# dealii-X/portable-multigrid

Measured on NVIDIA B200. Metric: GDoF/s of one multigrid V-cycle (fine-level DoFs / time); operator-apply GDoF/s in apply_gdofs, higher is better.
Workload: dtype f64

## Files before the change

### include/pmg_kernels.h

```cpp
#ifndef PMG_KERNELS_H
#define PMG_KERNELS_H

#include <stdint.h>

#ifdef __cplusplus
extern "C" {
#endif

#define PMGK_MAX_N1 10

typedef struct pmgk_level {
  int dim;
  int degree;
  int nx, ny, nz;
  int Nx, Ny, Nz;
  unsigned faces;
  int z0, nzl;
  int cz_lo, cz_hi;
  int z_own_lo, z_own_hi;
  double h[3];
  double S[PMGK_MAX_N1 * PMGK_MAX_N1];
  double lam[PMGK_MAX_N1];
  double Mref[PMGK_MAX_N1 * PMGK_MAX_N1];
  double Kref[PMGK_MAX_N1 * PMGK_MAX_N1];
  const double *dinv_tab;
  const double *dinv_vec;
  int tile_variant;
  const double *coef;
  int coef_cz0;
  double Sq[PMGK_MAX_N1 * PMGK_MAX_N1];
  double Dco[PMGK_MAX_N1 * PMGK_MAX_N1];
} pmgk_level;

enum { PMGK_APPLY = 0, PMGK_RESIDUAL = 1, PMGK_CHEB_FIRST = 2, PMGK_CHEB_STEP = 3 };

int pmgk_apply(const pmgk_level *lv, int mode, const double *u, const double *b, const double *xold,
               double *out, double f1, double f2, void *stream);
enum { PMGK_PART_ALL = 0, PMGK_PART_INTERIOR = 1, PMGK_PART_BOUNDARY = 2 };
int pmgk_apply_part(const pmgk_level *lv, int mode, const double *u, const double *b, const double *xold,
                    double *out, double f1, double f2, int part, void *stream);
int pmgk_apply_splits(const pmgk_level *lv, int mode);
typedef struct pmgk_push {
  double *out_lower, *out_upper;
  int lower_z0, upper_z0;
  void *mailbox, *mailbox_lower, *mailbox_upper;
  int push, consume;
} pmgk_push;
int pmgk_apply_push(const pmgk_level *lv, int mode, const double *u, const double *b, const double *xold,
                    double *out, double f1, double f2, const pmgk_push *push, void *stream);
int pmgk_apply_can_push(const pmgk_level *lv, int mode);
int pmgk_apply_geometry(const pmgk_level *lv, int *grid, int *block, int *smem_bytes, int *n_chunks);

int64_t pmgk_var_coef_doubles(const pmgk_level *lv);
int pmgk_var_fill_coef(const pmgk_level *lv, int kind, const double *gq, const double *gw, double *coef, void *stream);
int pmgk_var_fill_dinv(const pmgk_level *lv, const double *S2, const double *G2, double *dinv, void *stream);

int pmgk_fill_dinv(const pmgk_level *lv, double *dinv, void *stream);
int pmgk_scale_dinv(const pmgk_level *lv, double f, const double *b, double *out, void *stream);

int pmgk_set(double *x, double a, int64_t n, void *stream);
int pmgk_copy(double *dst, const double *src, int64_t n, void *stream);
int pmgk_axpby(double *out, double a, const double *x, double b, const double *y, int64_t n, void *stream);
int pmgk_scale(double *x, double a, int64_t n, void *stream);
int pmgk_dot(const double *x, const double *y, int64_t n, double *result, double *work, void *stream);
int pmgk_sum(const double *x, int64_t n, double *result, double *work, void *stream);
int pmgk_dot_work_doubles(void);
int pmgk_cg_update_xr(double *x, double *r, const double *p, const double *Ap, const double *alpha_dev,
                      int64_t n, double *result, double *work, void *stream);
int pmgk_cg_update_p(double *p, const double *z, const double *beta_dev, int64_t n, void *stream);
int pmgk_scalar_div(double *out, const double *num, const double *den, void *stream);
int pmgk_outer3(double *out, const double *lx, const double *ly, const double *lz, int Nx, int Ny, int nz, void *stream);
int pmgk_set_mod11(double *x, int64_t first_global, int64_t n, void *stream);

typedef struct pmgk_coarse_level {
  const pmgk_level *lv;
  int cheb_degree;
  double theta, delta;
  double *sol, *rhs, *tmp, *res;
} pmgk_coarse_level;
int pmgk_coarse_cycle_supported(const pmgk_level *lv);
int pmgk_coarse_cycle(const pmgk_coarse_level *levels, int n_levels, int pre, int post, const double *P1d_host, void *stream);

int pmgk_prolongate_and_add(int kind, const pmgk_level *coarse, const pmgk_level *fine, const double *P1d,
                            double *dst_fine, const double *src_coarse, void *stream);
// ... 18 lines not shown
```

### portable-multigrid_b200/csrc/pmg_apply.cu

```cuda
#include "pmg_apply_tile.h"
#include "pmg_cuda_common.h"
#include "pmg_kernels.h"

template <class Tile>
struct PmgDeviceExec {
  typename Tile::ThreadState st;
  template <class F> __device__ __forceinline__ void for_each_thread(F f) { f((int)threadIdx.x, st); }
  __device__ __forceinline__ void sync() { __syncthreads(); }
};

template <int P, int BX, int BY, int MINB>
__global__ void __launch_bounds__(PmgApplyTile<P, BX, BY>::NT, MINB)
pmg_apply_kernel(const __grid_constant__ PmgApplyParams<P> p)
{
  using Tile = PmgApplyTile<P, BX, BY>;
  extern __shared__ double pmg_smem[];
  PmgDeviceExec<Tile> ex;
  const int b = blockIdx.x;
  const int tile_x = b % p.tiles_x;
  const int tile_y = (b / p.tiles_x) % p.tiles_y;
  const int chunk = b / (p.tiles_x * p.tiles_y);
  Tile::run(p, ex, pmg_smem, tile_x, tile_y, chunk);
}

// ... 156 lines not shown
  if (mode != PMGK_APPLY && !b) return PMG_ERR_ARG;
  if (u == out) return PMG_ERR_ARG;
  return dispatch(lv, mode, u, b, xold, out, f1, f2, (cudaStream_t)stream, nullptr, part);
}

thread_local const pmgk_push *pmg_tl_push = nullptr;

static bool plane_kernel_level(const pmgk_level *lv)
{
  const bool small_level = small_level_of(lv);
  return lv->dim == 3 && !lv->coef && lv->degree <= PMG_PLANE_MAX_DEGREE && (lv->tile_variant == 6 || (lv->tile_variant == 0 && !small_level));
}

extern "C" int pmgk_apply_can_push(const pmgk_level *lv, int mode)
{
  return lv && (mode == PMGK_RESIDUAL || mode == PMGK_CHEB_FIRST || mode == PMGK_CHEB_STEP) && plane_kernel_level(lv) && lv->cz_hi - lv->cz_lo >= 2;
}

extern "C" int pmgk_apply_push(const pmgk_level *lv, int mode, const double *u, const double *b, const double *xold,
                               double *out, double f1, double f2, const pmgk_push *push, void *stream)
{
  if (!lv || !u || !out || !push) return PMG_ERR_ARG;
  if (mode != PMGK_APPLY && !b) return PMG_ERR_ARG;
  if (u == out) return PMG_ERR_ARG;
  if (!pmgk_apply_can_push(lv, mode)) return PMG_ERR_UNSUPPORTED;
  pmg_tl_push = push;
  const int rc = dispatch(lv, mode, u, b, xold, out, f1, f2, (cudaStream_t)stream, nullptr);
  pmg_tl_push = nullptr;
  return rc;
}

extern "C" int pmgk_apply_splits(const pmgk_level *lv, int mode)
{
  int g[4] = {0, 0, 0, 0};
  if (!lv) return 0;
  return dispatch(lv, mode, (const double *)16, (const double *)16, nullptr, (double *)32, 0, 0, 0, g, PMGK_PART_INTERIOR) == 0;
}

extern "C" int pmgk_apply_geometry(const pmgk_level *lv, int *grid, int *block, int *smem_bytes, int *n_chunks)
{
  int g[4] = {0, 0, 0, 0};
  const int rc = dispatch(lv, 0, (const double *)8, nullptr, nullptr, (double *)16, 0, 0, 0, g);
  if (grid) *grid = g[0];
  if (block) *block = g[1];
  if (smem_bytes) *smem_bytes = g[2];
  if (n_chunks) *n_chunks = g[3];
  return rc;
}
```

### portable-multigrid_b200/csrc/pmg_apply_plane.h

```cpp
#pragma once
#include "pmg_apply_sweep.h"

#if defined(__CUDA_ARCH__)
#define PMG_OPAQUE_PTR(ptr) asm volatile("" : "+l"(ptr))
#else
#define PMG_OPAQUE_PTR(ptr) ((void)0)
#endif
PMG_HD double pmg_plane_ldg(const double *ptr)
{
#if defined(__CUDA_ARCH__)
  double v;
  asm volatile("ld.global.f64 %0, [%1];\n" : "=d"(v) : "l"(ptr) : "memory");
  return v;
#else
  return *ptr;
#endif
}
PMG_HD void pmg_plane_prefetch(const double *ptr, int level)
{
#if defined(__CUDA_ARCH__)
  if (level == 1) asm volatile("prefetch.global.L2 [%0];\n" ::"l"(ptr) : "memory");
  else asm volatile("prefetch.global.L1 [%0];\n" ::"l"(ptr) : "memory");
#else
  (void)ptr; (void)level;
#endif
}
PMG_HD void pmg_plane_cp_async8(double *smem, unsigned base32, unsigned byte_off, const double *src_global)
{
#if defined(__CUDA_ARCH__)
  (void)smem;
  asm volatile("cp.async.ca.shared.global [%0], [%1], 8;\n" ::"r"(base32 + byte_off), "l"(src_global) : "memory");
#else
  (void)base32;
  *(double *)((char *)smem + byte_off) = *src_global;
#endif
}
struct alignas(16) PmgPlanePair { double c, d; };

#if defined(__CUDA_ARCH__)
#define PMG_KEEP(v) asm volatile("" : "+r"(v))
#else
#define PMG_KEEP(v) ((void)0)
#endif
PMG_HD void pmg_plane_stg(double *ptr, double v)
{
#if defined(__CUDA_ARCH__)
  asm volatile("st.global.f64 [%0], %1;\n" ::"l"(ptr), "d"(v) : "memory");
#else
  *ptr = v;
#endif
}

enum { PMG_FUSED_FROM_LO = 8, PMG_FUSED_FROM_HI = 9, PMG_FUSED_EPOCH_LO = 10, PMG_FUSED_EPOCH_HI = 11, PMG_FUSED_TICKET_LO = 12, PMG_FUSED_TICKET_HI = 13,
       PMG_FUSED_ERROR = 14  };

template <int P, int BX, int BY, int NT_, int FM = -1, int UZ = 1, int LW_ = 0, int NU_ = 3, int EPF = 0, int PR = 1, int XS = 1, int PUSH = 0>
struct PmgPlaneTile {
  static constexpr int N1 = P + 1;
  static constexpr int NT = NT_;
  static constexpr int MODE_STEP0 = 4;
  static PMG_HD int mode_of(const PmgSweepParams<P> &p)
  {
    return FM >= 0 ? FM : (p.mode == PMG_MODE_CHEB_STEP && p.xold == nullptr) ? MODE_STEP0 : p.mode;
  }
  static constexpr int OX = BX * P, OY = BY * P;
  static constexpr int XW = OX + P + 1, YW = OY + P + 1;
  static constexpr int UP = XW;
  static constexpr int UPLANE = YW * UP;
  static constexpr int CP = OY | 1;
// ... 399 lines not shown
    }
    if (DIR && t.xextra && tid < ERW) {
      const int gy = t.cy0 * P + tid;
      if (gy < p.Ny && (tid < OY || (!t.virt_y && gy == p.Ny - 1))) {
        const int64_t g = eoff + (int64_t)tid * p.Nx + OX;
        const double uc = pmg_plane_ldg(p.u + g);
        const double bb = (MODE != PMG_MODE_APPLY) ? pmg_plane_ldg(p.b + g) : 0.0;
        const double xo = has_xo ? pmg_plane_ldg(p.xold + g) : 0.0;
        pmg_plane_stg(p.out + g, epi_value<MODE>(p, 0.0, uc, bb, xo, true, 1.0));
      }
    }
  }
  template <int MODE>
  static PMG_HD void epilogue_m(const PmgSweepParams<P> &p, const TileGeom &t, const ThreadState &st, const double *smem, int slot,
                                int gz, int64_t eoff, int tid)
  {
    if (t.dirxy || gz == t.zlo || gz == t.zhi) epilogue_t<MODE, true>(p, t, st, smem, slot, gz, eoff, tid);
    else epilogue_t<MODE, false>(p, t, st, smem, slot, gz, eoff, tid);
  }
  static PMG_HD void epilogue(const PmgSweepParams<P> &p, const TileGeom &t, const ThreadState &st, const double *smem, int slot,
                              int gz, int64_t eoff, int tid)
  {
    switch (mode_of(p)) {
      case PMG_MODE_APPLY: epilogue_m<PMG_MODE_APPLY>(p, t, st, smem, slot, gz, eoff, tid); break;
      case PMG_MODE_RESIDUAL: epilogue_m<PMG_MODE_RESIDUAL>(p, t, st, smem, slot, gz, eoff, tid); break;
      case PMG_MODE_CHEB_FIRST: epilogue_m<PMG_MODE_CHEB_FIRST>(p, t, st, smem, slot, gz, eoff, tid); break;
      case PMG_MODE_CHEB_STEP: epilogue_m<PMG_MODE_CHEB_STEP>(p, t, st, smem, slot, gz, eoff, tid); break;
      default: epilogue_m<MODE_STEP0>(p, t, st, smem, slot, gz, eoff, tid); break;
    }
  }

  struct March {
    int cz_first, cz_begin, cz_end;
    bool top;
    int cur;
    int us;
    int gz_last;
    int gz_stop;
    int fetch_max;
    int q_lo, q_hi;
    int64_t eq;
    unsigned base32;
  };
  struct Plan { int n; int q[2]; int os[2]; };
  static PMG_HD Plan plan_of(const March &mc, int gz)
  {
    Plan pl; pl.n = 0;
    const int q = gz - P - 1;
    if (q >= mc.q_lo && q < mc.q_hi) {
      const int lay = q / P, k = q - lay * P;
      pl.q[0] = q; pl.os[0] = (k == P - 1) ? P - 1 + ((lay + 1) & 1) : k; pl.n = 1;
    }
    if (mc.top && gz == mc.gz_stop) { pl.q[pl.n] = mc.cz_end * P; pl.os[pl.n] = NOB - 1; ++pl.n; }
    return pl;
  }

  template <bool GEN, class Exec>
  static PMG_HD void layer(const PmgSweepParams<P> &p, const TileGeom &t, Exec &ex, double *smem, March &mc, int L)
  {
    double *Ub = smem + U_OFFSET, *Cb = smem + C_OFFSET, *Ob = smem + O_OFFSET;
    const bool prev_layer = L > mc.cz_first, emit_layer = L - 1 >= mc.cz_begin;
#pragma unroll(UZ ? P : 1)
    for (int jz = 0; jz < P; ++jz) {
      const int gz = L * P + jz;
      if (GEN && gz > mc.gz_stop) break;
      const bool last = GEN && (gz == mc.gz_last);
      const bool drain = GEN && (gz > mc.gz_last);
      const bool zero = GEN && (gz == t.zlo || gz == t.zhi);
      const bool fetch = gz + ND <= mc.fetch_max;
      int fs = mc.us + ND; if (fs >= NU) fs -= NU;
      double *Ucur = Ub + mc.us * UPLANE;
      double *Ccur = Cb + mc.cur * 2 * CPLANE;
      Plan pl;
      if (GEN) pl = plan_of(mc, gz);
      else {
        const int q = gz - P - 1;
        pl.n = (q >= mc.q_lo && q < mc.q_hi) ? 1 : 0; pl.q[0] = q; pl.q[1] = 0; pl.os[1] = 0;
        pl.os[0] = (P == 1) ? ((L - 1) & 1) : (jz == 0) ? P - 1 + ((L - 1) & 1) : jz - 1;
      }
      ex.for_each_thread([&](int, ThreadState &st) {
        load_plane(p, st, t.plane, smem, mc.base32, fs, fetch);
        if (pl.n > 0 && !drain) epi_issue(p, t, st, pl.q[0], mc.eq);
        if (!zero && !drain) ysweep(p, st, Ucur, Ccur);
        load_wait();
      });
      ex.sync();
      ex.for_each_thread([&](int tid, ThreadState &st) {
        const bool has_prev = (jz == 0) && prev_layer;
        if (!drain) xzsweep(p, st, Ccur, Ob, jz, zero, has_prev, !last, has_prev && emit_layer, last && mc.top, L & 1);
#pragma unroll
        for (int i = 0; i < 2; ++i)
          if (i < pl.n) {
            const int64_t eo = mc.eq + (int64_t)(pl.q[i] - (gz - P - 1)) * t.plane;
            if (drain || i > 0) epi_issue(p, t, st, pl.q[i], eo);
            epilogue(p, t, st, smem, pl.os[i], pl.q[i], eo, tid);
          }
      });
      mc.cur ^= 1;
      mc.us = (mc.us + 1 == NU) ? 0 : mc.us + 1;
      mc.eq += t.plane;
    }
  }

  template <class Exec>
  static PMG_HD void run(const PmgSweepParams<P> &p, Exec &ex, double *smem, int tile_x, int tile_y, int chunk)
  {
    const TileGeom t = geom(p, tile_x, tile_y);
    March mc;
    mc.cz_begin = p.cz_lo + chunk * p.layers_per_chunk;
    mc.cz_end = mc.cz_begin + p.layers_per_chunk;
    if (mc.cz_end > p.cz_hi) mc.cz_end = p.cz_hi;
    if (mc.cz_begin >= mc.cz_end) return;
    const bool halo = (mc.cz_begin > 0) && ((mc.cz_begin - 1) * P >= p.z0);
    mc.cz_first = halo ? mc.cz_begin - 1 : mc.cz_begin;
    mc.top = (mc.cz_end == p.cz_hi) && (mc.cz_end * P < p.z_own_hi);
    const int gz_first = mc.cz_first * P;
    mc.cur = 0; mc.us = 0;
#if defined(__CUDA_ARCH__)
    mc.base32 = (unsigned)__cvta_generic_to_shared(smem);
    PMG_KEEP(mc.base32);
#else
    mc.base32 = 0;
#endif
    mc.gz_last = mc.cz_end * P;
    mc.gz_stop = mc.gz_last + P;
    mc.fetch_max = (t.zhi >= 0 && t.zhi <= mc.gz_last) ? t.zhi - 1 : mc.gz_last;
    mc.q_lo = mc.cz_begin * P > p.z_own_lo ? mc.cz_begin * P : p.z_own_lo;
    mc.q_hi = mc.cz_end * P < p.z_own_hi ? mc.cz_end * P : p.z_own_hi;
    mc.eq = (int64_t)(gz_first - P - 1 - p.z0) * t.plane + t.tile0;
    const double *up = p.u + (int64_t)(gz_first - p.z0) * t.plane;

    int l_wait = -1;
    if constexpr (PUSH != 0)
      if (mc.gz_last >= p.z_own_hi && p.z_own_hi < p.Nz && (p.consume & 1) && p.mb_hi) {
        l_wait = (p.z_own_hi - ND) / P;
        if (l_wait <= mc.cz_first) { ex.wait_flag(p.mb, PMG_FUSED_FROM_HI, PMG_FUSED_EPOCH_HI); l_wait = -1; }
      }
    ex.for_each_thread([&](int tid, ThreadState &st) { decode(p, t, tid, st, smem); st.ld_src = up + st.ld_off; });
    ex.sync();
    ex.for_each_thread([&](int, ThreadState &st) {
#pragma unroll
      for (int d = 0; d < ND; ++d) {
        const int gz = gz_first + d;
        load_plane(p, st, t.plane, smem, mc.base32, d, gz <= mc.fetch_max && gz != t.zlo);
      }
      load_wait();
    });
    ex.sync();
    for (int L = mc.cz_first; L * P <= mc.gz_stop; ++L) {
      if constexpr (PUSH != 0)
        if (L == l_wait) ex.wait_flag(p.mb, PMG_FUSED_FROM_HI, PMG_FUSED_EPOCH_HI);
      const bool fast = L < mc.cz_end && L * P > t.zlo && (t.zhi < 0 || L * P + P - 1 < t.zhi);
      if (fast) layer<false>(p, t, ex, smem, mc, L);
      else layer<true>(p, t, ex, smem, mc, L);
    }
  }
  template <class Exec>
  static PMG_HD void push_boundary(const PmgSweepParams<P> &p, Exec &ex, int tile_x, int tile_y, bool at_lo, bool at_hi)
  {
    const int x0 = tile_x * OX, y0 = tile_y * OY;
    const int x1 = (tile_x == p.tiles_x - 1 || x0 + OX > p.Nx) ? p.Nx : x0 + OX;
    const int y1 = (tile_y == p.tiles_y - 1 || y0 + OY > p.Ny) ? p.Ny : y0 + OY;
    if (x0 >= x1 || y0 >= y1) return;
    const int w = x1 - x0, n = w * (y1 - y0);
    const int64_t plane = (int64_t)p.Nx * p.Ny;
    ex.sync();
    ex.for_each_thread([&](int tid, ThreadState &) {
      if (at_lo && p.push_lo) {
        const int64_t base = (int64_t)(p.z_own_lo - p.z0) * plane;
        for (int e = tid; e < n; e += NT) {
          const int r = e / w, c = e - r * w;
          const int64_t g = base + (int64_t)(y0 + r) * p.Nx + x0 + c;
          p.push_lo[g] = p.out[g];
        }
      }
      if (at_hi && p.push_hi) {
        for (int q = p.z_own_hi - P; q < p.z_own_hi; ++q) {
          const int64_t base = (int64_t)(q - p.z0) * plane;
          for (int e = tid; e < n; e += NT) {
            const int r = e / w, c = e - r * w;
            const int64_t g = base + (int64_t)(y0 + r) * p.Nx + x0 + c;
            p.push_hi[g] = p.out[g];
          }
        }
      }
// ... 9 lines not shown
```

### portable-multigrid_b200/csrc/pmg_apply_plane_launch.h

```cpp
#include "pmg_apply_plane.h"
#include "pmg_cuda_common.h"
#include "pmg_kernels.h"

namespace {

__device__ __forceinline__ void pmg_st_release_sys(unsigned long long *p, unsigned long long v)
{
  asm volatile("st.release.sys.global.u64 [%0], %1;\n" ::"l"(p), "l"(v) : "memory");
}
__device__ __forceinline__ unsigned long long pmg_ld_acquire_sys(const unsigned long long *p)
{
  unsigned long long v;
  asm volatile("ld.acquire.sys.global.u64 %0, [%1];\n" : "=l"(v) : "l"(p) : "memory");
  return v;
}

template <class Tile>
struct PmgPlaneDeviceExec {
  typename Tile::ThreadState st;
  template <class F> __device__ __forceinline__ void for_each_thread(F f) { f((int)threadIdx.x, st); }
  __device__ __forceinline__ void sync() { __syncthreads(); }
  __device__ __forceinline__ void wait_flag(unsigned long long *mb, int flag, int epoch)
  {
    if (threadIdx.x == 0) {
      const unsigned long long e = pmg_ld_acquire_sys(mb + epoch);
      if (pmg_ld_acquire_sys(mb + flag) < e) {
        const long long t0 = clock64();
        while (pmg_ld_acquire_sys(mb + flag) < e && pmg_ld_acquire_sys(mb + PMG_FUSED_ERROR) == 0) {
          __nanosleep(100);
          if (clock64() - t0 > 8000000000ll) { atomicExch(mb + PMG_FUSED_ERROR, 1ull); break; }
        }
      }
    }
    __syncthreads();
  }
};

template <int P, int BX, int BY, int NT, int MINB, int UZ, int FM, int PR, int XS, int PUSH>
__global__ void __launch_bounds__(NT, MINB)
pmg_plane_kernel(const __grid_constant__ PmgSweepParams<P> p, int chunk_first, int chunk_stride)
{
  using Tile = PmgPlaneTile<P, BX, BY, NT, FM, UZ, 0, 3, 0, PR, XS, PUSH>;
  extern __shared__ __align__(128) double pmg_plane_smem[];
  PmgPlaneDeviceExec<Tile> ex;
  const int b = blockIdx.x;
  const int tile_x = b % p.tiles_x;
  const int tile_y = (b / p.tiles_x) % p.tiles_y;
  const int group = b / (p.tiles_x * p.tiles_y);
  int chunk = chunk_first + group * chunk_stride;
  bool at_lo = false, at_hi = false;
  if (PUSH && p.mb) {
    const int last = p.n_chunks - 1;
    if (!(p.consume & 2)) chunk = group == 0 ? last : group == last ? 0 : group;
    at_lo = chunk == 0; at_hi = chunk == last;
    if (at_lo && (p.consume & 1) && p.mb_lo) ex.wait_flag(p.mb, PMG_FUSED_FROM_LO, PMG_FUSED_EPOCH_LO);
  }
  Tile::run(p, ex, pmg_plane_smem, tile_x, tile_y, chunk);
  if (!PUSH || !(at_lo || at_hi)) return;
  Tile::push_boundary(p, ex, tile_x, tile_y, at_lo, at_hi);
  __syncthreads();
  if (threadIdx.x == 0) {
    if (p.consume & 8) __threadfence(); else if (!(p.consume & 4)) __threadfence_system();
    const unsigned long long tiles = (unsigned long long)p.tiles_x * p.tiles_y;
    if (at_lo && atomicAdd(p.mb + PMG_FUSED_TICKET_LO, 1ull) == tiles - 1) {
      p.mb[PMG_FUSED_TICKET_LO] = 0;
      const unsigned long long e = pmg_ld_acquire_sys(p.mb + PMG_FUSED_EPOCH_LO) + 1;
      __threadfence_system();
      if (p.mb_lo) pmg_st_release_sys(p.mb_lo + PMG_FUSED_FROM_HI, e);
      pmg_st_release_sys(p.mb + PMG_FUSED_EPOCH_LO, e);
    }
    if (at_hi && atomicAdd(p.mb + PMG_FUSED_TICKET_HI, 1ull) == tiles - 1) {
      p.mb[PMG_FUSED_TICKET_HI] = 0;
      const unsigned long long e = pmg_ld_acquire_sys(p.mb + PMG_FUSED_EPOCH_HI) + 1;
      __threadfence_system();
      if (p.mb_hi) pmg_st_release_sys(p.mb_hi + PMG_FUSED_FROM_LO, e);
      pmg_st_release_sys(p.mb + PMG_FUSED_EPOCH_HI, e);
    }
  }
}

inline void choose_plane_chunks(int tiles, int layers, int slots, int degree, int *n_chunks, int *layers_per_chunk)
{
  const long c_target = (8L * slots + tiles - 1) / tiles;
  const long c_fill = (slots + tiles - 1) / tiles;
  const int lpc_min = (32 + degree - 1) / degree;
  long c_cap = layers / lpc_min;
  long c_fill_cap = layers / 2;
  if (c_cap < 1) c_cap = 1;
  if (c_fill_cap < 1) c_fill_cap = 1;
  long c_floor = c_fill < c_fill_cap ? c_fill : c_fill_cap;
  if (c_floor < c_cap) c_floor = c_cap;
  long c = c_target < c_floor ? c_target : c_floor;
  if (c < 1) c = 1;
  const int lpc = (layers + (int)c - 1) / (int)c;
  *layers_per_chunk = lpc;
  *n_chunks = (layers + lpc - 1) / lpc;
}

template <int P, int BX, int BY, int NT, int MINB, int UZ, int FM, int PR, int XS, int PUSH>
int launch_plane(const pmgk_level *lv, const double *u, const double *b, const double *xold, double *out, double f1, double f2,
                 cudaStream_t stream, int *geom, int part)
{
  using Tile = PmgPlaneTile<P, BX, BY, NT, FM, UZ, 0, 3, 0, PR, XS, PUSH>;
  auto kernel = pmg_plane_kernel<P, BX, BY, NT, MINB, UZ, FM, PR, XS, PUSH>;
  PmgSweepParams<P> p;
  p.nx = lv->nx; p.ny = lv->ny; p.nz = lv->nz;
  p.Nx = lv->Nx; p.Ny = lv->Ny; p.Nz = lv->Nz;
  p.faces = lv->faces;
  p.z0 = lv->z0; p.nzl = lv->nzl;
  p.cz_lo = lv->cz_lo; p.cz_hi = lv->cz_hi;
  p.z_own_lo = lv->z_own_lo; p.z_own_hi = lv->z_own_hi;
  p.tiles_x = Tile::tiles_of(lv->nx, lv->faces >> 1 & 1u, BX);
  p.tiles_y = Tile::tiles_of(lv->ny, lv->faces >> 3 & 1u, BY);
  const int smem_bytes = Tile::SMEM_DOUBLES * (int)sizeof(double);
  enum { MAXDEV = 64 };
  static int ctas_per_sm[MAXDEV];
  int dev = 0;
  PMG_CUDA_CHECK(cudaGetDevice(&dev));
  if (dev < 0 || dev >= MAXDEV) return PMG_ERR_UNSUPPORTED;
  int per_sm = __atomic_load_n(&ctas_per_sm[dev], __ATOMIC_ACQUIRE);
  if (per_sm == 0) {
    PMG_CUDA_CHECK(cudaFuncSetAttribute(kernel, cudaFuncAttributeMaxDynamicSharedMemorySize, smem_bytes));
    PMG_CUDA_CHECK(cudaOccupancyMaxActiveBlocksPerMultiprocessor(&per_sm, kernel, NT, smem_bytes));
    if (per_sm < 1) return PMG_ERR_CUDA;
    __atomic_store_n(&ctas_per_sm[dev], per_sm, __ATOMIC_RELEASE);
  }
  const int slots = pmgk_device_sm_count() * per_sm;
  choose_plane_chunks(p.tiles_x * p.tiles_y, lv->cz_hi - lv->cz_lo, slots, P, &p.n_chunks, &p.layers_per_chunk);
  pmg_sweep_fill_matrices<P>(p, lv->Mref, lv->Kref, lv->h);
  p.mode = (FM == 4) ? PMG_MODE_CHEB_STEP : FM; p.u = u; p.b = b; p.xold = xold; p.out = out; p.f1 = f1; p.f2 = f2;
  p.dinv_vec = lv->dinv_vec; p.dinv_tab = lv->dinv_tab;
  p.push_lo = p.push_hi = nullptr; p.mb = p.mb_lo = p.mb_hi = nullptr; p.consume = 0;
  if (const pmgk_push *ps = PUSH ? pmg_tl_push : nullptr) {
    if (part != PMGK_PART_ALL || lv->cz_hi - lv->cz_lo < 2 || !ps->mailbox) return PMG_ERR_UNSUPPORTED;
    const int64_t plane = (int64_t)lv->Nx * lv->Ny;
    if (ps->push && ps->out_lower) p.push_lo = ps->out_lower + plane * (lv->z0 - ps->lower_z0);
    if (ps->push && ps->out_upper) p.push_hi = ps->out_upper + plane * (lv->z0 - ps->upper_z0);
    p.mb = (unsigned long long *)ps->mailbox;
    p.mb_lo = (unsigned long long *)ps->mailbox_lower; p.mb_hi = (unsigned long long *)ps->mailbox_upper;
    p.consume = ps->consume;
  }
  int chunk_first = 0, chunk_stride = 1, chunk_count = p.n_chunks;
  if (part != PMGK_PART_ALL) {
    if (p.n_chunks < 3) return PMG_ERR_UNSUPPORTED;
    if (part == PMGK_PART_INTERIOR) { chunk_first = 1; chunk_count = p.n_chunks - 2; }
    else { chunk_stride = p.n_chunks - 1; chunk_count = 2; }
  }
  const int grid = p.tiles_x * p.tiles_y * chunk_count;
  if (geom) { geom[0] = grid; geom[1] = NT; geom[2] = smem_bytes; geom[3] = p.n_chunks; return 0; }
  if ((int64_t)lv->Nx * lv->Ny * 4 >= (int64_t)1 << 31) return PMG_ERR_UNSUPPORTED;
  kernel<<<grid, NT, smem_bytes, stream>>>(p, chunk_first, chunk_stride);
  PMG_CUDA_CHECK(cudaGetLastError());
  pmg_count_launch(1);
  return 0;
}

}

#define PMG_PLANE_CAT2(a, b) a##b
#define PMG_PLANE_CAT(a, b) PMG_PLANE_CAT2(a, b)

int PMG_PLANE_CAT(pmg_plane_dispatch_m, PMG_PLANE_TU_MODE)(const pmgk_level *lv, const double *u, const double *b, const double *xold,
                                                           double *out, double f1, double f2, cudaStream_t s, int *geom, int part)
{
  switch (lv->degree) {
#if PMG_PLANE_TU_MODE >= 1
#define PMG_PLANE_LAUNCH(P, BX, BY, NT, MINB, UZ, PR, XS)                                                                              \
  case P:                                                                                                                             \
    return pmg_tl_push ? launch_plane<P, BX, BY, NT, MINB, UZ, PMG_PLANE_TU_MODE, PR, XS, 1>(lv, u, b, xold, out, f1, f2, s, geom, part) \
                       : launch_plane<P, BX, BY, NT, MINB, UZ, PMG_PLANE_TU_MODE, PR, XS, 0>(lv, u, b, xold, out, f1, f2, s, geom, part);
#else
#define PMG_PLANE_LAUNCH(P, BX, BY, NT, MINB, UZ, PR, XS) \
  case P: return pmg_tl_push ? PMG_ERR_UNSUPPORTED : launch_plane<P, BX, BY, NT, MINB, UZ, PMG_PLANE_TU_MODE, PR, XS, 0>(lv, u, b, xold, out, f1, f2, s, geom, part);
#endif
#if PMG_PLANE_TU_MODE == 0
#define PMG_PLANE_CASE(P, BX, BY, NT, MINB, UZ, PR, XS) PMG_PLANE_LAUNCH(P, BX, BY, NT, MINB, UZ, PR, XS)
#define PMG_PLANE_CASE_F(P, BX, BY, NT, MINB, UZ, PR, XS)
#else
#define PMG_PLANE_CASE(P, BX, BY, NT, MINB, UZ, PR, XS)
#define PMG_PLANE_CASE_F(P, BX, BY, NT, MINB, UZ, PR, XS) PMG_PLANE_LAUNCH(P, BX, BY, NT, MINB, UZ, PR, XS)
#endif
#include "pmg_apply_plane_tiles.inc"
#undef PMG_PLANE_CASE
// ... 6 lines not shown
```

### portable-multigrid_b200/csrc/pmg_apply_sweep.h

```cpp
#pragma once
#include <stdint.h>
#include <math.h>

#if defined(__CUDACC__)
#define PMG_HD __host__ __device__ __forceinline__
#else
#define PMG_HD inline
#endif

#ifndef PMG_APPLY_MODES_DEFINED
#define PMG_APPLY_MODES_DEFINED
enum PmgApplyMode {
  PMG_MODE_APPLY = 0,
  PMG_MODE_RESIDUAL = 1,
  PMG_MODE_CHEB_FIRST = 2,
  PMG_MODE_CHEB_STEP = 3,
};
#endif

PMG_HD void pmg_mbar_init(uint64_t *bar, int count)
{
#if defined(__CUDA_ARCH__)
  asm volatile("mbarrier.init.shared::cta.b64 [%0], %1;\n" ::"r"((unsigned)__cvta_generic_to_shared(bar)), "r"(count) : "memory");
#else
// ... 47 lines not shown
{
#if defined(__CUDA_ARCH__)
  asm volatile("cp.async.bulk.shared::cluster.global.mbarrier::complete_tx::bytes [%0], [%1], %2, [%3];\n"
               ::"r"((unsigned)__cvta_generic_to_shared(dst_smem)), "l"(src_global), "r"(bytes),
                 "r"((unsigned)__cvta_generic_to_shared(bar)) : "memory");
#else
  (void)bar;
  for (int i = 0; i < bytes / 8; ++i) dst_smem[i] = src_global[i];
#endif
}

template <int P>
struct PmgSweepParams {
  int nx, ny, nz;
  int Nx, Ny, Nz;
  unsigned faces;
  int z0, nzl;
  int cz_lo, cz_hi;
  int z_own_lo, z_own_hi;
  int tiles_x, tiles_y, n_chunks, layers_per_chunk;
  double M[(P + 1) * (P + 1)], Kx[(P + 1) * (P + 1)], Ky[(P + 1) * (P + 1)];
  double Mz[(P + 1) * (P + 1)], Kz[(P + 1) * (P + 1)];
  int mode;
  const double *u;
  const double *b;
  const double *xold;
  double *out;
  double f1, f2;
  const double *dinv_vec;
  const double *dinv_tab;
  double *push_lo, *push_hi;
  unsigned long long *mb, *mb_lo, *mb_hi;
  int consume;
};

template <int P>
inline void pmg_sweep_fill_matrices(PmgSweepParams<P> &p, const double *Mref, const double *Kref, const double *h)
{
  constexpr int N1 = P + 1;
  const double cx = h[1] * h[2] / h[0], cy = h[0] * h[2] / h[1], cz = h[0] * h[1] / h[2];
  for (int i = 0; i < N1; ++i)
    for (int j = 0; j < N1; ++j) {
      const int a = i * N1 + j, b = j * N1 + i, c = (P - i) * N1 + (P - j), d = (P - j) * N1 + (P - i);
      const double m = 0.25 * (Mref[a] + Mref[b] + Mref[c] + Mref[d]);
      const double k = 0.25 * (Kref[a] + Kref[b] + Kref[c] + Kref[d]);
      p.M[a] = m; p.Kx[a] = k; p.Ky[a] = (cy / cx) * k; p.Mz[a] = cx * m; p.Kz[a] = cz * k;
    }
}

template <int P>
PMG_HD int pmg_sweep_pos_type(int g, int N)
{
  return (g == 0) ? P : (g == N - 1) ? P + 1 : g % P;
}

template <int P>
PMG_HD constexpr int pmg_sweep_canon(int i, int j)
{
  int m = i * (P + 1) + j;
  const int b = j * (P + 1) + i, c = (P - i) * (P + 1) + (P - j), d = (P - j) * (P + 1) + (P - i);
  if (b < m) m = b;
  if (c < m) m = c;
  if (d < m) m = d;
  return m;
}

// ... 631 lines not shown
```

### portable-multigrid_b200/host/pmg_internal.h

```cpp
#ifndef PMG_INTERNAL_H
#define PMG_INTERNAL_H

#include <cuda_runtime_api.h>
#include <nccl.h>
#include <stdint.h>
#include "pmg.h"
#include "pmg_kernels.h"

#ifdef __cplusplus
extern "C" {
#endif

void pmg_set_error(const char *fmt, ...);
void pmg_count_launch(int n);
int pmg_enter(const pmg_context *ctx);

#define PMG_CHECK(call)                        \
  do {                                         \
    int pmg_rc_ = (call);                      \
    if (pmg_rc_ != PMG_OK) return pmg_rc_;     \
  } while (0)

#define PMG_CUDA(call)                                                                            \
  do {                                                                                            \
// ... 83 lines not shown
  int gathered;
  int cz_lo, cz_hi;
  int z0, nzl;
  int z_own_lo, z_own_hi;
  int lower, upper;
  int64_t plane;
  int64_t n_local;
  int64_t n_global;
} pmg_layout;

int pmg_p2p_init(pmg_context *ctx);
void pmg_p2p_shutdown(pmg_context *ctx);
int pmg_p2p_register(pmg_context *ctx, const pmg_layout *lay, double *d);
double *pmg_p2p_acquire(pmg_context *ctx, const pmg_layout *lay);
int pmg_p2p_release(pmg_context *ctx, double *d);
int pmg_p2p_halo(pmg_context *ctx, const pmg_layout *lay, double *d, cudaStream_t stream, int *done);
void pmg_p2p_forget(pmg_context *ctx);
int pmg_p2p_push_desc(pmg_context *ctx, const pmg_layout *lay, double *out, pmgk_push *desc);

struct pmg_vector {
  pmg_context *ctx;
  pmg_layout lay;
  double *d;
  int borrowed;
};

struct pmg_operator {
  pmg_context *ctx;
  int dim, degree, coefficient;
  unsigned faces;
  pmg_layout lay;
  pmgk_level lv;
  double *d_dinv_tab;
  double *d_coef;
  pmg_vector *dinv;
  pmg_vector *cg_ws[4];
};

struct pmg_transfer {
  pmg_context *ctx;
  int kind;
  const pmg_operator *coarse, *fine;
  double *d_P;
  double *d_scratch;
  pmg_vector *gather_buf;
};

struct pmg_chebyshev {
  pmg_operator *op;
  double smoothing_range;
  int degree, eig_cg_n_iterations;
  int initialized;
  double lambda_min, lambda_max, theta, delta;
  int cg_iterations;
  pmg_vector *t0, *t1;
};

int pmg_layout_make(pmg_context *ctx, int dim, int degree, int nx, int ny, int nz, pmg_layout *lay);
int pmg_layout_same(const pmg_layout *a, const pmg_layout *b);
int pmg_vector_create_layout(pmg_context *ctx, const pmg_layout *lay, pmg_vector **v);
int pmg_halo_update(pmg_context *ctx, const pmg_layout *lay, double *d);
int pmg_halo_update_on(pmg_context *ctx, const pmg_layout *lay, double *d, ncclComm_t comm, cudaStream_t stream);
int pmg_allreduce_sum(pmg_context *ctx, double *dev_scalar, int count);
int pmg_vector_dot_device(const pmg_vector *x, const pmg_vector *y, int slot);
int pmg_apply_with_halo(const pmg_operator *op, int mode, double *u, const double *b, const double *xold, double *out, double f1, double f2);
int pmg_apply_chain_ok(const pmg_operator *op, int mode, double *v0, double *v1);
// ... 13 lines not shown
```

### portable-multigrid_b200/host/pmg_operator.c

```c
#include "pmg_internal.h"
#include <math.h>
#include <stdlib.h>
#include <string.h>

static int var_diagonal(pmg_operator *op)
{
  const int n1 = op->degree + 1;
  double Sq[PMGK_MAX_N1 * PMGK_MAX_N1], G[PMGK_MAX_N1 * PMGK_MAX_N1];
  pmg_fe_shape_tables(op->degree, Sq, NULL, G, NULL, NULL);
  for (int i = 0; i < n1 * n1; ++i) { Sq[i] *= Sq[i]; G[i] *= G[i]; }
  return pmgk_var_fill_dinv(&op->lv, Sq, G, op->dinv->d, op->ctx->stream);
}

static int setup_coefficient(pmg_operator *op)
{
  pmgk_level *lv = &op->lv;
  double gq[PMGK_MAX_N1], gw[PMGK_MAX_N1];
  pmg_fe_shape_tables(op->degree, lv->Sq, lv->Dco, NULL, gq, gw);
  lv->coef_cz0 = lv->z0 / op->degree;
  PMG_CHECK(pmg_vector_create_layout(op->ctx, &op->lay, &op->dinv));
  if (!op->lay.active) return PMG_OK;
  const int64_t n = pmgk_var_coef_doubles(lv);
  if (cudaMalloc((void **)&op->d_coef, sizeof(double) * (size_t)n) != cudaSuccess) {
    pmg_set_error("cudaMalloc of %lld coefficient values failed", (long long)n);
// ... 19 lines not shown
  pmg_operator *op = (pmg_operator *)calloc(1, sizeof(*op));
  if (!op) return PMG_ERR_NOMEM;
  op->ctx = ctx; op->dim = dim; op->degree = degree; op->coefficient = coefficient; op->faces = faces & PMG_ALL_FACES;
  PMG_CHECK(pmg_layout_make(ctx, dim, degree, nx, ny, nz, &op->lay));
  pmgk_level *lv = &op->lv;
  lv->dim = dim;
  lv->degree = degree;
  lv->nx = nx; lv->ny = ny; lv->nz = nz;
  lv->Nx = op->lay.Nx; lv->Ny = op->lay.Ny; lv->Nz = op->lay.Nz;
  lv->faces = op->faces;
  lv->z0 = op->lay.z0; lv->nzl = op->lay.nzl;
  lv->cz_lo = op->lay.cz_lo; lv->cz_hi = op->lay.cz_hi;
  lv->z_own_lo = op->lay.z_own_lo; lv->z_own_hi = op->lay.z_own_hi;
  lv->h[0] = 1.0 / nx; lv->h[1] = 1.0 / ny; lv->h[2] = (dim == 2) ? 1.0 : 1.0 / nz;
  pmg_fe_fastdiag(degree, lv->S, lv->lam);
  pmg_fe_pencil(degree, lv->Mref, lv->Kref);
  const int T = degree + 2;
  double *tab = (double *)malloc(sizeof(double) * T * T * T);
  if (!tab) { free(op); return PMG_ERR_NOMEM; }
  pmg_fe_dinv_table(degree, lv->h, dim, tab);
  PMG_CUDA(cudaSetDevice(ctx->device));
  PMG_CUDA(cudaMalloc((void **)&op->d_dinv_tab, sizeof(double) * T * T * T));
  PMG_CUDA(cudaMemcpyAsync(op->d_dinv_tab, tab, sizeof(double) * T * T * T, cudaMemcpyHostToDevice, ctx->stream));
  PMG_CUDA(cudaStreamSynchronize(ctx->stream));
  free(tab);
  lv->dinv_tab = op->d_dinv_tab;
  lv->dinv_vec = NULL;
  const char *tv = getenv("PMG_TILE_VARIANT");
  lv->tile_variant = tv ? atoi(tv) : 0;
  if (coefficient != 0) {
    const int rc = setup_coefficient(op);
    if (rc != PMG_OK) { pmg_laplace_operator_destroy(op); return rc; }
  }
  *out = op;
  return PMG_OK;
}

int pmg_laplace_operator_destroy(pmg_operator *op)
{
  if (!op) return PMG_OK;
  cudaStreamSynchronize(op->ctx->stream);
  if (op->dinv) pmg_vector_destroy(op->dinv);
  for (int i = 0; i < 4; ++i) if (op->cg_ws[i]) pmg_vector_destroy(op->cg_ws[i]);
  cudaFree(op->d_dinv_tab);
  cudaFree(op->d_coef);
  free(op);
  return PMG_OK;
}

static int check_vec(const pmg_operator *op, const pmg_vector *v, const char *what)
{
  if (!v || v->ctx != op->ctx || !pmg_layout_same(&v->lay, &op->lay)) {
    pmg_set_error("%s: vector is not initialised for this operator (initialize_dof_vector)", what);
    return PMG_ERR_ARG;
  }
  return PMG_OK;
}

static int fused_order_bit(void)
{
  static int natural_order = -1;
  if (natural_order < 0) { const char *e = getenv("PMG_FUSED_ORDER"); natural_order = (e && atoi(e) == 1) ? 0 : 1; }
  return natural_order ? 2 : 0;
}

int pmg_apply_with_halo(const pmg_operator *op, int mode, double *u, const double *b, const double *xold, double *out, double f1, double f2)
{
  if (op) PMG_CHECK(pmg_enter(op->ctx));
  pmg_context *ctx = op->ctx;
  if (!op->lay.active) return PMG_OK;
  const int slab = ctx->has_comm && !op->lay.gathered;
  if (slab && ctx->overlap && pmgk_apply_splits(&op->lv, mode)) {
    PMG_CUDA(cudaEventRecord(ctx->ev_ready, ctx->stream));
    PMG_CUDA(cudaStreamWaitEvent(ctx->halo_stream, ctx->ev_ready, 0));
    PMG_CHECK(pmg_halo_update_on(ctx, &op->lay, u, ctx->halo_comm, ctx->halo_stream));
    PMG_CUDA(cudaEventRecord(ctx->ev_halo, ctx->halo_stream));
    PMG_CHECK(pmgk_apply_part(&op->lv, mode, u, b, xold, out, f1, f2, PMGK_PART_INTERIOR, ctx->stream));
// ... 234 lines not shown
```

Measured before the change: 3.118.

## Add dynamic persistent work-claiming scheduler for plane sweep kernel chunks

For non-push full applies, the plane kernel now launches at most one CTA per resident slot. Each CTA claims (tile, chunk) items from a global atomic counter in a staggered run order. When a CTA reaches the end of its chunk it can claim the next chunk of the same tile and keep marching, which reuses the plane data already in shared memory instead of reloading halo layers. Chunks are made shorter to give finer load balance. This adds atomic traffic, a grid-wide reset of the schedule table by the last CTA, and a per-operator device buffer.

```diff
diff --git a/include/pmg_kernels.h b/include/pmg_kernels.h
--- a/include/pmg_kernels.h
+++ b/include/pmg_kernels.h
@@ -25,6 +25,8 @@
   double Kref[PMGK_MAX_N1 * PMGK_MAX_N1];
   const double *dinv_tab;
   const double *dinv_vec;
+  int *plane_sched;
+  int64_t plane_sched_words;
   int tile_variant;
   const double *coef;
   int coef_cz0;
@@ -50,6 +52,7 @@
                     double *out, double f1, double f2, const pmgk_push *push, void *stream);
 int pmgk_apply_can_push(const pmgk_level *lv, int mode);
 int pmgk_apply_geometry(const pmgk_level *lv, int *grid, int *block, int *smem_bytes, int *n_chunks);
+int64_t pmgk_plane_sched_words(const pmgk_level *lv);
 
 int64_t pmgk_var_coef_doubles(const pmgk_level *lv);
 int pmgk_var_fill_coef(const pmgk_level *lv, int kind, const double *gq, const double *gw, double *coef, void *stream);
diff --git a/portable-multigrid_b200/csrc/pmg_apply.cu b/portable-multigrid_b200/csrc/pmg_apply.cu
--- a/portable-multigrid_b200/csrc/pmg_apply.cu
+++ b/portable-multigrid_b200/csrc/pmg_apply.cu
@@ -212,14 +212,28 @@
 
 extern "C" int pmgk_apply_splits(const pmgk_level *lv, int mode)
 {
-  int g[4] = {0, 0, 0, 0};
+  int g[5] = {0, 0, 0, 0, 0};
   if (!lv) return 0;
   return dispatch(lv, mode, (const double *)16, (const double *)16, nullptr, (double *)32, 0, 0, 0, g, PMGK_PART_INTERIOR) == 0;
 }
 
+extern "C" int64_t pmgk_plane_sched_words(const pmgk_level *lv)
+{
+  int64_t words = 0;
+  if (!lv) return 0;
+  for (int mode = PMGK_APPLY; mode <= PMGK_CHEB_STEP + 1; ++mode) {
+    int g[5] = {0, 0, 0, 0, 0};
+    const int m = mode > PMGK_CHEB_STEP ? PMGK_CHEB_STEP : mode;
+    if (dispatch(lv, m, (const double *)8, (const double *)8, mode == PMGK_CHEB_STEP ? (const double *)8 : nullptr, (double *)16, 0, 0, 0, g) == 0 &&
+        g[4] > words)
+      words = g[4];
+  }
+  return words;
+}
+
 extern "C" int pmgk_apply_geometry(const pmgk_level *lv, int *grid, int *block, int *smem_bytes, int *n_chunks)
 {
-  int g[4] = {0, 0, 0, 0};
+  int g[5] = {0, 0, 0, 0, 0};
   const int rc = dispatch(lv, 0, (const double *)8, nullptr, nullptr, (double *)16, 0, 0, 0, g);
   if (grid) *grid = g[0];
   if (block) *block = g[1];
diff --git a/portable-multigrid_b200/csrc/pmg_apply_plane.h b/portable-multigrid_b200/csrc/pmg_apply_plane.h
--- a/portable-multigrid_b200/csrc/pmg_apply_plane.h
+++ b/portable-multigrid_b200/csrc/pmg_apply_plane.h
@@ -1,4 +1,6 @@
 #pragma once
+#include <type_traits>
+#include <utility>
 #include "pmg_apply_sweep.h"
 
 #if defined(__CUDA_ARCH__)
@@ -35,6 +37,11 @@
   *(double *)((char *)smem + byte_off) = *src_global;
 #endif
 }
+template <class Exec, class Params, class = void> struct PmgPlaneClaims : std::false_type {};
+template <class Exec, class Params>
+struct PmgPlaneClaims<Exec, Params, std::void_t<decltype(std::declval<Exec &>().may_continue(std::declval<const Params &>(), 0, 0))>>
+    : std::true_type {};
+
 struct alignas(16) PmgPlanePair { double c, d; };
 
 #if defined(__CUDA_ARCH__)
@@ -500,26 +507,27 @@
 
   struct March {
     int cz_first, cz_begin, cz_end;
-    bool top;
     int cur;
     int us;
-    int gz_last;
-    int gz_stop;
-    int fetch_max;
-    int q_lo, q_hi;
+    int q_lo;
     int64_t eq;
     unsigned base32;
+    PMG_HD int gz_last() const { return cz_end * P; }
+    PMG_HD int gz_stop() const { return cz_end * P + P; }
+    PMG_HD int fetch_max(const TileGeom &t) const { return (t.zhi >= 0 && t.zhi <= gz_last()) ? t.zhi - 1 : gz_last(); }
+    PMG_HD int q_hi(const PmgSweepParams<P> &p) const { return cz_end * P < p.z_own_hi ? cz_end * P : p.z_own_hi; }
+    PMG_HD bool top(const PmgSweepParams<P> &p) const { return cz_end == p.cz_hi && cz_end * P < p.z_own_hi; }
   };
   struct Plan { int n; int q[2]; int os[2]; };
-  static PMG_HD Plan plan_of(const March &mc, int gz)
+  static PMG_HD Plan plan_of(const PmgSweepParams<P> &p, const March &mc, int gz)
   {
     Plan pl; pl.n = 0;
     const int q = gz - P - 1;
-    if (q >= mc.q_lo && q < mc.q_hi) {
+    if (q >= mc.q_lo && q < mc.q_hi(p)) {
       const int lay = q / P, k = q - lay * P;
       pl.q[0] = q; pl.os[0] = (k == P - 1) ? P - 1 + ((lay + 1) & 1) : k; pl.n = 1;
     }
-    if (mc.top && gz == mc.gz_stop) { pl.q[pl.n] = mc.cz_end * P; pl.os[pl.n] = NOB - 1; ++pl.n; }
+    if (mc.top(p) && gz == mc.gz_stop()) { pl.q[pl.n] = mc.cz_end * P; pl.os[pl.n] = NOB - 1; ++pl.n; }
     return pl;
   }
 
@@ -531,19 +539,19 @@
 #pragma unroll(UZ ? P : 1)
     for (int jz = 0; jz < P; ++jz) {
       const int gz = L * P + jz;
-      if (GEN && gz > mc.gz_stop) break;
-      const bool last = GEN && (gz == mc.gz_last);
-      const bool drain = GEN && (gz > mc.gz_last);
+      if (GEN && gz > mc.gz_stop()) break;
+      const bool last = GEN && (gz == mc.gz_last());
+      const bool drain = GEN && (gz > mc.gz_last());
       const bool zero = GEN && (gz == t.zlo || gz == t.zhi);
-      const bool fetch = gz + ND <= mc.fetch_max;
+      const bool fetch = !GEN || gz + ND <= mc.fetch_max(t);
       int fs = mc.us + ND; if (fs >= NU) fs -= NU;
       double *Ucur = Ub + mc.us * UPLANE;
       double *Ccur = Cb + mc.cur * 2 * CPLANE;
       Plan pl;
-      if (GEN) pl = plan_of(mc, gz);
+      if (GEN) pl = plan_of(p, mc, gz);
       else {
         const int q = gz - P - 1;
-        pl.n = (q >= mc.q_lo && q < mc.q_hi) ? 1 : 0; pl.q[0] = q; pl.q[1] = 0; pl.os[1] = 0;
+        pl.n = q >= mc.q_lo ? 1 : 0; pl.q[0] = q; pl.q[1] = 0; pl.os[1] = 0;
         pl.os[0] = (P == 1) ? ((L - 1) & 1) : (jz == 0) ? P - 1 + ((L - 1) & 1) : jz - 1;
       }
       ex.for_each_thread([&](int, ThreadState &st) {
@@ -555,7 +563,7 @@
       ex.sync();
       ex.for_each_thread([&](int tid, ThreadState &st) {
         const bool has_prev = (jz == 0) && prev_layer;
-        if (!drain) xzsweep(p, st, Ccur, Ob, jz, zero, has_prev, !last, has_prev && emit_layer, last && mc.top, L & 1);
+        if (!drain) xzsweep(p, st, Ccur, Ob, jz, zero, has_prev, !last, has_prev && emit_layer, last && mc.top(p), L & 1);
 #pragma unroll
         for (int i = 0; i < 2; ++i)
           if (i < pl.n) {
@@ -576,12 +584,9 @@
     const TileGeom t = geom(p, tile_x, tile_y);
     March mc;
     mc.cz_begin = p.cz_lo + chunk * p.layers_per_chunk;
-    mc.cz_end = mc.cz_begin + p.layers_per_chunk;
-    if (mc.cz_end > p.cz_hi) mc.cz_end = p.cz_hi;
-    if (mc.cz_begin >= mc.cz_end) return;
+    if (mc.cz_begin >= p.cz_hi) return;
     const bool halo = (mc.cz_begin > 0) && ((mc.cz_begin - 1) * P >= p.z0);
     mc.cz_first = halo ? mc.cz_begin - 1 : mc.cz_begin;
-    mc.top = (mc.cz_end == p.cz_hi) && (mc.cz_end * P < p.z_own_hi);
     const int gz_first = mc.cz_first * P;
     mc.cur = 0; mc.us = 0;
 #if defined(__CUDA_ARCH__)
@@ -590,17 +595,14 @@
 #else
     mc.base32 = 0;
 #endif
-    mc.gz_last = mc.cz_end * P;
-    mc.gz_stop = mc.gz_last + P;
-    mc.fetch_max = (t.zhi >= 0 && t.zhi <= mc.gz_last) ? t.zhi - 1 : mc.gz_last;
+    mc.cz_end = mc.cz_begin + p.layers_per_chunk < p.cz_hi ? mc.cz_begin + p.layers_per_chunk : p.cz_hi;
     mc.q_lo = mc.cz_begin * P > p.z_own_lo ? mc.cz_begin * P : p.z_own_lo;
-    mc.q_hi = mc.cz_end * P < p.z_own_hi ? mc.cz_end * P : p.z_own_hi;
     mc.eq = (int64_t)(gz_first - P - 1 - p.z0) * t.plane + t.tile0;
     const double *up = p.u + (int64_t)(gz_first - p.z0) * t.plane;
 
     int l_wait = -1;
     if constexpr (PUSH != 0)
-      if (mc.gz_last >= p.z_own_hi && p.z_own_hi < p.Nz && (p.consume & 1) && p.mb_hi) {
+      if (mc.gz_last() >= p.z_own_hi && p.z_own_hi < p.Nz && (p.consume & 1) && p.mb_hi) {
         l_wait = (p.z_own_hi - ND) / P;
         if (l_wait <= mc.cz_first) { ex.wait_flag(p.mb, PMG_FUSED_FROM_HI, PMG_FUSED_EPOCH_HI); l_wait = -1; }
       }
@@ -610,15 +612,23 @@
 #pragma unroll
       for (int d = 0; d < ND; ++d) {
         const int gz = gz_first + d;
-        load_plane(p, st, t.plane, smem, mc.base32, d, gz <= mc.fetch_max && gz != t.zlo);
+        load_plane(p, st, t.plane, smem, mc.base32, d, gz <= mc.fetch_max(t) && gz != t.zlo);
       }
       load_wait();
     });
     ex.sync();
-    for (int L = mc.cz_first; L * P <= mc.gz_stop; ++L) {
+    static_assert(ND <= P + 1, "the continuation is decided before the first plane above the march is fetched");
+    const int tile = tile_y * p.tiles_x + tile_x;
+    constexpr bool claims = PmgPlaneClaims<Exec, PmgSweepParams<P>>::value;
+    for (int L = mc.cz_first; L * P <= mc.gz_stop(); ++L) {
       if constexpr (PUSH != 0)
         if (L == l_wait) ex.wait_flag(p.mb, PMG_FUSED_FROM_HI, PMG_FUSED_EPOCH_HI);
-      const bool fast = L < mc.cz_end && L * P > t.zlo && (t.zhi < 0 || L * P + P - 1 < t.zhi);
+      if constexpr (claims)
+        if (L == mc.cz_end - 1 && mc.cz_end < p.cz_hi && ex.may_continue(p, tile, ++chunk)) {
+          const int cz_end = mc.cz_end + p.layers_per_chunk;
+          mc.cz_end = cz_end < p.cz_hi ? cz_end : p.cz_hi;
+        }
+      const bool fast = L < mc.cz_end - 1 && L * P > t.zlo && (t.zhi < 0 || L * P + P - 1 + ND < t.zhi);
       if (fast) layer<false>(p, t, ex, smem, mc, L);
       else layer<true>(p, t, ex, smem, mc, L);
     }
diff --git a/portable-multigrid_b200/csrc/pmg_apply_plane_launch.h b/portable-multigrid_b200/csrc/pmg_apply_plane_launch.h
--- a/portable-multigrid_b200/csrc/pmg_apply_plane_launch.h
+++ b/portable-multigrid_b200/csrc/pmg_apply_plane_launch.h
@@ -15,11 +15,24 @@
   return v;
 }
 
-template <class Tile>
+__shared__ int pmg_plane_item;
+
+template <class Tile, bool DYN>
 struct PmgPlaneDeviceExec {
   typename Tile::ThreadState st;
   template <class F> __device__ __forceinline__ void for_each_thread(F f) { f((int)threadIdx.x, st); }
   __device__ __forceinline__ void sync() { __syncthreads(); }
+  template <class Params>
+  __device__ __forceinline__ bool may_continue(const Params &p, int, int)
+  {
+    if (!DYN || !p.sched) return false;
+    int ok = 0;
+    if (threadIdx.x == 0) {
+      ok = atomicExch(p.sched + pmg_plane_item + 1, 1) == 0;
+      if (ok) ++pmg_plane_item;
+    }
+    return __syncthreads_or(ok);
+  }
   __device__ __forceinline__ void wait_flag(unsigned long long *mb, int flag, int epoch)
   {
     if (threadIdx.x == 0) {
@@ -36,16 +49,40 @@
   }
 };
 
+template <class Params>
+__device__ __forceinline__ int pmg_plane_next_item(const Params &p)
+{
+  int *const sched = p.sched;
+  const int tiles = p.tiles_x * p.tiles_y, C = p.n_chunks, R = p.sched_runs, G = p.sched_run_len;
+  const int starts = tiles * R, n = starts * G;
+  for (;;) {
+    const int idx = atomicAdd(sched + tiles * C, 1);
+    if (idx >= n) return -1;
+    int j, chunk;
+    if (idx < starts) {
+      const int q = idx / tiles;
+      j = idx - q * tiles;
+      const int r = (j + q) % R;
+      chunk = r * G;
+    } else {
+      const int e = idx - starts, d = G - 1 - e / starts, rem = e % starts;
+      const int r = rem / tiles;
+      j = rem - r * tiles;
+      chunk = r * G + d;
+    }
+    if (chunk < C && atomicExch(sched + j * C + chunk, 1) == 0) return j * C + chunk;
+  }
+}
+
 template <int P, int BX, int BY, int NT, int MINB, int UZ, int FM, int PR, int XS, int PUSH>
 __global__ void __launch_bounds__(NT, MINB)
 pmg_plane_kernel(const __grid_constant__ PmgSweepParams<P> p, int chunk_first, int chunk_stride)
 {
   using Tile = PmgPlaneTile<P, BX, BY, NT, FM, UZ, 0, 3, 0, PR, XS, PUSH>;
   extern __shared__ __align__(128) double pmg_plane_smem[];
-  PmgPlaneDeviceExec<Tile> ex;
+  PmgPlaneDeviceExec<Tile, PUSH == 0> ex;
   const int b = blockIdx.x;
-  const int tile_x = b % p.tiles_x;
-  const int tile_y = (b / p.tiles_x) % p.tiles_y;
+  int tile = b % (p.tiles_x * p.tiles_y);
   const int group = b / (p.tiles_x * p.tiles_y);
   int chunk = chunk_first + group * chunk_stride;
   bool at_lo = false, at_hi = false;
@@ -55,8 +92,33 @@
     at_lo = chunk == 0; at_hi = chunk == last;
     if (at_lo && (p.consume & 1) && p.mb_lo) ex.wait_flag(p.mb, PMG_FUSED_FROM_LO, PMG_FUSED_EPOCH_LO);
   }
-  Tile::run(p, ex, pmg_plane_smem, tile_x, tile_y, chunk);
+  const bool dynamic = PUSH == 0 && p.sched;
+  for (;;) {
+    if (dynamic) {
+      if (threadIdx.x == 0) pmg_plane_item = pmg_plane_next_item(p);
+      __syncthreads();
+      const int it = pmg_plane_item;
+      if (it < 0) break;
+      tile = it / p.n_chunks;
+      chunk = it - tile * p.n_chunks;
+    }
+    Tile::run(p, ex, pmg_plane_smem, tile % p.tiles_x, tile / p.tiles_x, chunk);
+    if (!dynamic) break;
+  }
+  if (dynamic) {
+    const int tiles = p.tiles_x * p.tiles_y;
+    int last = 0;
+    if (threadIdx.x == 0) {
+      __threadfence();
+      last = atomicAdd(p.sched + tiles * p.n_chunks + 1, 1) == (int)gridDim.x - 1;
+      if (last) __threadfence();
+    }
+    if (__syncthreads_or(last))
+      for (int e = threadIdx.x; e < tiles * p.n_chunks + 2; e += NT) p.sched[e] = 0;
+    return;
+  }
   if (!PUSH || !(at_lo || at_hi)) return;
+  const int tile_x = tile % p.tiles_x, tile_y = tile / p.tiles_x;
   Tile::push_boundary(p, ex, tile_x, tile_y, at_lo, at_hi);
   __syncthreads();
   if (threadIdx.x == 0) {
@@ -93,6 +155,17 @@
   long c = c_target < c_floor ? c_target : c_floor;
   if (c < 1) c = 1;
   const int lpc = (layers + (int)c - 1) / (int)c;
+  *layers_per_chunk = lpc;
+  *n_chunks = (layers + lpc - 1) / lpc;
+}
+
+enum { PMG_PLANE_CLAIM_STEPS = 16 };
+inline void plane_claim_chunks(int tiles, int layers, int slots, int degree, int *n_chunks, int *layers_per_chunk)
+{
+  int lpc = (PMG_PLANE_CLAIM_STEPS + degree - 1) / degree;
+  const int c_fill = (slots + tiles - 1) / tiles;
+  if ((layers + lpc - 1) / lpc < c_fill) lpc = layers / c_fill > 1 ? layers / c_fill : 1;
+  if (lpc > layers) lpc = layers;
   *layers_per_chunk = lpc;
   *n_chunks = (layers + lpc - 1) / lpc;
 }
@@ -126,7 +199,10 @@
     __atomic_store_n(&ctas_per_sm[dev], per_sm, __ATOMIC_RELEASE);
   }
   const int slots = pmgk_device_sm_count() * per_sm;
-  choose_plane_chunks(p.tiles_x * p.tiles_y, lv->cz_hi - lv->cz_lo, slots, P, &p.n_chunks, &p.layers_per_chunk);
+  const int tiles = p.tiles_x * p.tiles_y, layers = lv->cz_hi - lv->cz_lo;
+  const bool dynamic = PUSH == 0 && part == PMGK_PART_ALL;
+  if (dynamic) plane_claim_chunks(tiles, layers, slots, P, &p.n_chunks, &p.layers_per_chunk);
+  else choose_plane_chunks(tiles, layers, slots, P, &p.n_chunks, &p.layers_per_chunk);
   pmg_sweep_fill_matrices<P>(p, lv->Mref, lv->Kref, lv->h);
   p.mode = (FM == 4) ? PMG_MODE_CHEB_STEP : FM; p.u = u; p.b = b; p.xold = xold; p.out = out; p.f1 = f1; p.f2 = f2;
   p.dinv_vec = lv->dinv_vec; p.dinv_tab = lv->dinv_tab;
@@ -146,9 +222,24 @@
     if (part == PMGK_PART_INTERIOR) { chunk_first = 1; chunk_count = p.n_chunks - 2; }
     else { chunk_stride = p.n_chunks - 1; chunk_count = 2; }
   }
-  const int grid = p.tiles_x * p.tiles_y * chunk_count;
-  if (geom) { geom[0] = grid; geom[1] = NT; geom[2] = smem_bytes; geom[3] = p.n_chunks; return 0; }
+  int grid = tiles * chunk_count;
+  p.sched = nullptr; p.sched_runs = p.sched_run_len = 0;
+  const int64_t sched_words = dynamic ? (int64_t)tiles * p.n_chunks + 2 : 0;
+  if (dynamic) {
+    const int C = p.n_chunks;
+    int R = (slots + tiles - 1) / tiles;
+    if (R < 2) R = 2;
+    if (R > C) R = C;
+    p.sched_run_len = (C + R - 1) / R;
+    p.sched_runs = (C + p.sched_run_len - 1) / p.sched_run_len;
+    if (grid > slots) grid = slots;
+  }
+  if (geom) { geom[0] = grid; geom[1] = NT; geom[2] = smem_bytes; geom[3] = p.n_chunks; geom[4] = (int)sched_words; return 0; }
   if ((int64_t)lv->Nx * lv->Ny * 4 >= (int64_t)1 << 31) return PMG_ERR_UNSUPPORTED;
+  if (dynamic) {
+    if (!lv->plane_sched || lv->plane_sched_words < sched_words) return PMG_ERR_UNSUPPORTED;
+    p.sched = lv->plane_sched;
+  }
   kernel<<<grid, NT, smem_bytes, stream>>>(p, chunk_first, chunk_stride);
   PMG_CUDA_CHECK(cudaGetLastError());
   pmg_count_launch(1);
diff --git a/portable-multigrid_b200/csrc/pmg_apply_sweep.h b/portable-multigrid_b200/csrc/pmg_apply_sweep.h
--- a/portable-multigrid_b200/csrc/pmg_apply_sweep.h
+++ b/portable-multigrid_b200/csrc/pmg_apply_sweep.h
@@ -103,6 +103,8 @@
   double *push_lo, *push_hi;
   unsigned long long *mb, *mb_lo, *mb_hi;
   int consume;
+  int *sched;
+  int sched_runs, sched_run_len;
 };
 
 template <int P>
diff --git a/portable-multigrid_b200/host/pmg_internal.h b/portable-multigrid_b200/host/pmg_internal.h
--- a/portable-multigrid_b200/host/pmg_internal.h
+++ b/portable-multigrid_b200/host/pmg_internal.h
@@ -139,6 +139,7 @@
   pmg_layout lay;
   pmgk_level lv;
   double *d_dinv_tab;
+  int *d_plane_sched;
   double *d_coef;
   pmg_vector *dinv;
   pmg_vector *cg_ws[4];
diff --git a/portable-multigrid_b200/host/pmg_operator.c b/portable-multigrid_b200/host/pmg_operator.c
--- a/portable-multigrid_b200/host/pmg_operator.c
+++ b/portable-multigrid_b200/host/pmg_operator.c
@@ -75,6 +75,18 @@
     const int rc = setup_coefficient(op);
     if (rc != PMG_OK) { pmg_laplace_operator_destroy(op); return rc; }
   }
+  const int64_t sched_words = op->lay.active ? pmgk_plane_sched_words(lv) : 0;
+  if (sched_words > 0) {
+    if (cudaMalloc((void **)&op->d_plane_sched, sizeof(int) * (size_t)sched_words) != cudaSuccess) {
+      pmg_set_error("cudaMalloc of %lld scheduling words failed", (long long)sched_words);
+      pmg_laplace_operator_destroy(op);
+      return PMG_ERR_NOMEM;
+    }
+    PMG_CUDA(cudaMemsetAsync(op->d_plane_sched, 0, sizeof(int) * (size_t)sched_words, ctx->stream));
+    PMG_CUDA(cudaStreamSynchronize(ctx->stream));
+    lv->plane_sched = op->d_plane_sched;
+    lv->plane_sched_words = sched_words;
+  }
   *out = op;
   return PMG_OK;
 }
@@ -86,6 +98,7 @@
   if (op->dinv) pmg_vector_destroy(op->dinv);
   for (int i = 0; i < 4; ++i) if (op->cg_ws[i]) pmg_vector_destroy(op->cg_ws[i]);
   cudaFree(op->d_dinv_tab);
+  cudaFree(op->d_plane_sched);
   cudaFree(op->d_coef);
   free(op);
   return PMG_OK;
```

Result: slower. 2.517, median of 6 (-19.3%).
